# ajzhai/PEANUT

Hardware: AMD Instinct MI355X
Metric: maps/sec for 480x480x(4+N_cat) prediction fwd, batch 32 (higher is better)
Workload: dtype f32; 1 GPU; 480x480, 14-channel (4+10) partial maps -> 6-class prediction forward (PSPNet R50-V1c-D8), batch 32 per GPU, seeded random-init weights; survey_config=2, global_batch=32, parallelism=dp1 (map shards, no data-path collective)

## Files before the change

### peanut_amd/csrc/common.h

```cpp
#pragma once
#include <hip/hip_runtime.h>
#include <stdint.h>
#include <string>

namespace peanut {

void set_error(const std::string& msg);
int fail(int code, const std::string& msg);
void note_kernel(const char* family);
const char* noted_kernel();

#define PEANUT_HIP_CHECK(expr)                                                            \
  do {                                                                                    \
    hipError_t _e = (expr);                                                               \
    if (_e != hipSuccess)                                                                 \
      return ::peanut::fail(-3, std::string(#expr) + ": " + hipGetErrorString(_e));       \
  } while (0)

struct ConvDesc {
  int cin;
  int cout;
  int kh, kw, stride, pad, dil;
  int relu;
  int bn_tile;
// ... 49 lines not shown
#pragma clang fp contract(off)
  const float gx = ((float)x + 0.5f - bx[0]) / (bx[2] - bx[0]) * 2.f - 1.f;
  const float gy = ((float)y + 0.5f - bx[1]) / (bx[3] - bx[1]) * 2.f - 1.f;
  const float ix = ((gx + 1.f) * (float)M - 1.f) / 2.f, iy = ((gy + 1.f) * (float)M - 1.f) / 2.f;
  const float fx = floorf(ix), fy = floorf(iy);
  const int x0 = (int)fminf(fmaxf(fx, -2.f), (float)M + 1.f), y0 = (int)fminf(fmaxf(fy, -2.f), (float)M + 1.f);
  if (x0 < -1 || x0 >= M || y0 < -1 || y0 >= M) return 0.f;
  const float lx = ix - fx, ly = iy - fy;
  const float wx = 1.f - lx, wy = 1.f - ly;
  auto at = [&](int yy, int xx) -> float {
    return ((unsigned)yy < (unsigned)M && (unsigned)xx < (unsigned)M) ? m[yy * M + xx] : 0.f;
  };
  return at(y0, x0) * wy * wx + at(y0, x0 + 1) * wy * lx + at(y0 + 1, x0) * ly * wx + at(y0 + 1, x0 + 1) * ly * lx;
}

inline int conv_out_dim(int n, int k, int s, int p, int d) { return (n + 2 * p - d * (k - 1) - 1) / s + 1; }

void conv_pick_tiles(int cin_pad, int cout, int* bn_tile, int* bk, bool pointwise = false);
size_t conv_packed_floats(int cin_pad, int cout, int kh, int kw, int bn_tile);
void pack_conv_weights(const float* w_oihw, int cout, int cin_real, int cin_pad, int kh, int kw,
                       int bn_tile, int bk, float* out);
int launch_conv(const ConvDesc& d, const ConvArgs& a, hipStream_t stream);
bool conv_pw_enabled();
bool conv_pw_uses_256(int cout, long long M, int mt_per_group, int bn_tile, int cin);
int conv_pw_256_min_k();
bool conv_pw_uses_256w(int cout, long long M, int mt_per_group, int bn_tile, int cin, int flush_ktiles);
bool conv_pw_narrow_tiles(int cin, int cout, long long M, int bn_tile, int mt_per_group);
bool conv_pw_uses_256p(int cout, long long M, int mt_per_group, int bn_tile, int cin, int flush_ktiles, long long in_pixels = 0);
struct ConvKParams;
bool gemm_skinny_takes(const ConvKParams& p, int bn_tile, size_t ws_floats);
int launch_gemm_skinny(const ConvKParams& p, float* ws, size_t ws_floats, hipStream_t stream);
bool conv_pw_uses_256wp(int cout, long long M, int stride, int mt_per_group, int bn_tile, int c1, int c2, int flush_ktiles);
bool conv_pw_uses_ares(int cin, int cout, long long M, int stride, bool two_source, int flush_ktiles, int bn_tile);

bool conv_patch_eligible(const ConvDesc& d, const ConvArgs& a);
const char* conv_patch_kernel_name(const ConvDesc& d, bool nchw);
bool conv_patch_nchw_eligible(const ConvDesc& d, int B, int Ho, int Wo, int creal);
int launch_conv_patch_nchw(const ConvDesc& d, const float* x_nchw, int creal, float* y, int B, int H, int W, int Ho, int Wo, hipStream_t stream);

void wino_geometry(int B, int H, int W, int dil, int* th, int* tw, long long* n_tiles, long long* m_pad, int gran = 128, int m = 4);
void wino_transform_weights(const float* w_oihw, int cout, int cin, float* out, int m = 4);
int launch_wino_input(const float* x, float* V, int B, int H, int W, int C, int dil, hipStream_t s, int gran = 128, int m = 4, long long m_pad_total = 0,
                      const DeferredSplit* df = nullptr);
bool wino_input_accepts_deferred(int B, int H, int W, int C, int dil, int gran, int m);
long long wino_deferred_count();
int launch_wino_output(const float* Mb, const float* scale, const float* shift, const float* res, float* y,
                       int B, int H, int W, int C, int dil, int relu, hipStream_t s, int gran = 128, int m = 4, long long m_pad_total = 0);

bool gemm_rs_uses_256(int cout, long long M, int mt_per_group, int bn_tile, int cin);
const char* gemm_rs_kernel_name(int cout, long long M, int mt_per_group, int bn_tile, int cin, int planes);
size_t sx_packed_bytes(int cin_pad, int cout, int bn_tile, int planes);
void pack_weights_sx(const float* w, int cout, int cin_real, int cin_pad, int bn_tile, int planes, float wscale, void* out);
float sx_pack_scale(const float* w, size_t n, int planes);
size_t sx_conv_packed_bytes(int cin_pad, int cout, int kh, int kw, int bn_tile, int planes);
void pack_weights_sx_conv(const float* w_oihw, int cout, int cin_real, int cin_pad, int kh, int kw, int bn_tile, int planes,
                          float wscale, void* out);

int launch_nchw_to_nhwc_pad(const float* x, float* y, int B, int C, int H, int W, int Cpad, hipStream_t s);
int launch_maxpool3x3s2(const float* x, float* y, int B, int H, int W, int C, int Ho, int Wo, hipStream_t s);
int launch_ppm_pool(const float* x, float* out, int B, int H, int W, int C, const int* scales, int nscales,
                    hipStream_t s, int scale_rows = 0);
size_t ppm_pool_scratch_floats(int B, int H, int C, const int* scales, int nscales);
int launch_ppm_pool2(const float* x, float* scratch, float* out, int B, int H, int W, int C, const int* scales,
                     int nscales, hipStream_t s, int scale_rows = 0);
int launch_ppm_upsample_concat(const float* table, float* out, int B, int H, int W, int Cp, const int* scales,
                               int nscales, int align_corners, hipStream_t s);
// ... 7 lines not shown
```

### peanut_amd/csrc/conv_common.h

```cpp
#pragma once
#include <stdlib.h>

#include <atomic>

#include "common.h"
#include "options.h"

namespace peanut {

typedef float f32x16 __attribute__((ext_vector_type(16)));
typedef float f32x4 __attribute__((ext_vector_type(4)));

__device__ __forceinline__ float relu_keep_nan(float v) { return v < 0.f ? 0.f : v; }
__device__ __forceinline__ f32x4 relu_keep_nan(f32x4 v) {
  return f32x4{relu_keep_nan(v.x), relu_keep_nan(v.y), relu_keep_nan(v.z), relu_keep_nan(v.w)};
}

struct ConvKParams {
  const float* x;
  const float* x2;
  const float* w;
  const float* scale;
  const float* shift;
  const float* res;
// ... 14 lines not shown
  int ares_pbn;
  int phase_shift;
  int sk_units, sk_maxp, sk_g, sk_q;
  int pack_bn;
  int group_valid;
  int p_order;
  float* dump;
  int stagger;
  int flush;
  DeferredSplit* defer;
  const int* group_rows;
};

template <int I>
struct IC { static constexpr int value = I; };
template <int N, int I = 0, class F>
__device__ __forceinline__ void static_for(F&& f) {
  if constexpr (I < N) {
    f(IC<I>{});
    static_for<N, I + 1>(f);
  }
}

struct KIter {
  int tap, ky, kx, cbase;
  const float* wtile;
};


const float* zero_page();
bool conv_pw_enabled();
int launch_conv_pw(const ConvKParams& p, int bn_tile, float* ws, size_t ws_floats, hipStream_t stream);
int launch_conv_pw_ares(const ConvKParams& p, int bn_tile, hipStream_t stream);
int launch_conv_pw256p(const ConvKParams& p, float* ws, size_t ws_floats, hipStream_t stream);
int launch_conv_pw256wp(const ConvKParams& p, float* ws, size_t ws_floats, hipStream_t stream);
int launch_conv_patch(const ConvKParams& p, const ConvDesc& d, int B, hipStream_t stream);
int launch_gemm_rs(const ConvKParams& p, int bn_tile, int planes, float* ws, size_t ws_floats, hipStream_t stream);
int launch_conv_rs(const ConvKParams& p, int bn_tile, int planes, float* ws, size_t ws_floats, hipStream_t stream);


struct Work { int mt, nt, kt0, kt1, item; };

__host__ __device__ __forceinline__ int sk_owner(long long U, int G, long long u) {
  int w = (int)(u * G / U);
  while (w + 1 < G && U * (w + 1) / G <= u) ++w;
  while (w > 0 && U * w / G > u) --w;
  return w;
}

__device__ __forceinline__ void tile_to_mn(const ConvKParams& p, int tile, int* mt_out, int* nt_out) {
  int mt, nt;
  if (p.nchunk > 0 && p.ntiles > p.nchunk) {
    const int full = p.ntiles / p.nchunk, rem = p.ntiles - full * p.nchunk;
    const int per_chunk = p.mtiles * p.nchunk;
    if (tile < full * per_chunk) {
      const int c = tile / per_chunk, r = tile - c * per_chunk;
      mt = r / p.nchunk;
      nt = c * p.nchunk + (r - mt * p.nchunk);
    } else {
      const int r = tile - full * per_chunk;
      mt = r / rem;
      nt = full * p.nchunk + (r - mt * rem);
    }
  } else {
    mt = tile / p.ntiles;
    nt = tile - mt * p.ntiles;
// ... 212 lines not shown
    for (int s = 1; s < parts; ++s) v += *reinterpret_cast<const f32x4*>(base + (size_t)s * (BM * BN) + row * BN + c4);
    const int ss_off = (p.mt_per_group && p.ss_group_stride) ? (mt / p.mt_per_group) * p.ss_group_stride : 0;
    const f32x4 sc = *reinterpret_cast<const f32x4*>(p.scale + ss_off + n) * p.alpha;
    const f32x4 sh = *reinterpret_cast<const f32x4*>(p.shift + ss_off + n);
#pragma unroll
    for (int e = 0; e < 4; ++e) v[e] = __builtin_fmaf(v[e], sc[e], sh[e]);
    const size_t o = (size_t)m * p.cout + n;
    if (vec_ok) {
      if (n < p.cout) {
        if (p.res) v += *reinterpret_cast<const f32x4*>(p.res + o);
        if (p.relu) v = relu_keep_nan(v);
        *reinterpret_cast<f32x4*>(p.y + o) = v;
      }
    } else {
      for (int e = 0; e < 4; ++e) {
        if (n + e < p.cout) {
          float x = v[e];
          if (p.res) x += p.res[o + e];
          if (p.relu) x = relu_keep_nan(x);
          p.y[o + e] = x;
        }
      }
    }
  }
}

struct SlotCache {
  static constexpr int kMaxDevices = 16;
  std::atomic<int> slots[kMaxDevices];
  std::atomic<int> cus[kMaxDevices];
  SlotCache() { for (int i = 0; i < kMaxDevices; ++i) { slots[i].store(0); cus[i].store(0); } }
};

template <typename KernelT, int BM, int BN, int NT = 256>
int launch_with_tail_split(KernelT kernel, ConvKParams p, float* ws, size_t ws_floats, hipStream_t stream, SlotCache* cache) {
  int dev = 0;
  if (hipGetDevice(&dev) != hipSuccess || dev < 0 || dev >= SlotCache::kMaxDevices) return fail(-3, "conv launch: no current device");
  int slots = cache->slots[dev].load(std::memory_order_relaxed), cus = cache->cus[dev].load(std::memory_order_relaxed);
  if (slots == 0) {
    int occ = 0;
    if (hipDeviceGetAttribute(&cus, hipDeviceAttributeMultiprocessorCount, dev) != hipSuccess ||
        hipOccupancyMaxActiveBlocksPerMultiprocessor(&occ, kernel, NT, 0) != hipSuccess || occ < 1)
      slots = -1;
    else
      slots = cus * occ;
    cache->cus[dev].store(cus, std::memory_order_relaxed);
    cache->slots[dev].store(slots, std::memory_order_relaxed);
  }
  const int mtiles = (p.M + BM - 1) / BM;
  const int T = mtiles * p.ntiles;
  int sp = 1;
  const int t = plan_tail_split(T, slots, cus, p.nkt, (size_t)BM * BN, ws ? ws_floats : 0, &sp);
  p.split_p = sp;
  p.n_sp = t * sp;
  p.n_full = T - t;
  p.partial = ws;
  p.mtiles = mtiles;
  p.nchunk = (int)opt(OPT_NCHUNK);
  p.res_prefetch = opt(OPT_RES_PREFETCH) != 0;
  bool deferred = false;
  if (p.defer) {
    DeferredSplit* df = p.defer;
    if (BM == 128 && BN == 128 && t > 0 && t == T && !p.res && p.mt_per_group == 0 && p.cout % 128 == 0 &&
        !(p.nchunk > 0 && p.ntiles > p.nchunk)) {
      df->valid = true;
      df->partial = ws; df->split_p = sp; df->ntiles = p.ntiles; df->M = p.M; df->cout = p.cout; df->relu = p.relu;
      df->scale = p.scale; df->shift = p.shift; df->alpha = p.alpha;
      deferred = true;
    }
    p.defer = nullptr;
  }
  hipLaunchKernelGGL(kernel, dim3((unsigned)(p.n_full + p.n_sp)), dim3(NT), 0, stream, p);
  if (t > 0 && !deferred) hipLaunchKernelGGL((conv_splitk_reduce_kernel<BM, BN>), dim3((unsigned)t, BM / 16), dim3(256), 0, stream, p);
  hipError_t e = hipGetLastError();
  if (e != hipSuccess) return fail(-3, std::string("conv launch: ") + hipGetErrorString(e));
  return 0;
}

}
```

### peanut_amd/csrc/conv_pw.hip

```cpp
#include <stdlib.h>

#include "common.h"
#include "conv_common.h"

namespace peanut {

namespace {

typedef const __attribute__((address_space(1))) void* gptr_t;
typedef __attribute__((address_space(3))) void* lptr_t;

template <int BN, int WM, int WN>
__global__ __launch_bounds__(256) __attribute__((amdgpu_waves_per_eu(BN == 128 ? 2 : (BN == 64 ? 3 : 4))))
void conv_pw_glds_kernel(const ConvKParams p) {
  constexpr int BM = 128, BK = 32;
  constexpr int TM = BM / WM, TN = BN / WN;
  constexpr int MI = TM / 32, NI = TN / 32;
  constexpr int A_FLOATS = BM * BK, B_FLOATS = BN * BK, STAGE = A_FLOATS + B_FLOATS;
  constexpr int A_INSTR = BM / 32, B_INSTR = BN / 32;
  constexpr int CS = BN + 4;
  constexpr int EP = (BM * CS > 2 * STAGE) ? WM : 1;
  constexpr int ER = BM / EP;
  constexpr int SMEM_FLOATS = (2 * STAGE > ER * CS) ? 2 * STAGE : ER * CS;
  static_assert(WM * WN == 4 && TM % 32 == 0 && TN % 32 == 0, "4 waves, wave tile a multiple of 32x32");
// ... 357 lines not shown
    _Pragma("unroll") for (int t = 0; t < MI; ++t) af[j][t] = *reinterpret_cast<const f32x4*>(cur + a_row + t * 32 * BK + sw[(g) + j]); \
    _Pragma("unroll") for (int u = 0; u < NI; ++u) bf[j][u] = *reinterpret_cast<const f32x4*>(cur + b_row + u * 32 * BK + sw[(g) + j]); \
  }
#define PW256W_MFMA_PAIR()                                                                                \
  _Pragma("unroll") for (int j = 0; j < 2; ++j)                                                           \
    _Pragma("unroll") for (int kk = 0; kk < 4; ++kk)                                                      \
      _Pragma("unroll") for (int t = 0; t < MI; ++t)                                                      \
        _Pragma("unroll") for (int u = 0; u < NI; ++u)                                                    \
          acc[t][u] = __builtin_amdgcn_mfma_f32_32x32x2f32(af[j][t][kk], bf[j][u][kk], acc[t][u], 0, 0, 0);
  for (int kt = 0; kt < nk; ++kt) {
    const float* const cur = smem + (kt & 1) * STAGE;
    float* const fill = smem + ((kt + 1) & 1) * STAGE;
    const bool more = kt + 1 < nk;
    if (more && !late) PW256W_DMA_TILE(fill);
    f32x4 af[2][MI], bf[2][NI];
    PW256W_READ_PAIR(0);
    PW256W_MFMA_PAIR();
    __builtin_amdgcn_sched_barrier(0);
    if (more && late) PW256W_DMA_TILE(fill);
    __builtin_amdgcn_sched_barrier(0);
    PW256W_READ_PAIR(2);
    PW256W_MFMA_PAIR();
    asm volatile("s_waitcnt vmcnt(0)" ::: "memory");
    PW256W_BARRIER();
  }
#undef PW256W_DMA_TILE
#undef PW256W_BARRIER
#undef PW256W_READ_PAIR
#undef PW256W_MFMA_PAIR
  conv_epilogue<BM, BN, WM, WN, WM, NT>(p, wk, acc, smem, m0, n0);
}

template <int BN, int WM, int WN>
int launch_pw_t(const ConvKParams& p, float* ws, size_t ws_floats, hipStream_t stream) {
  static SlotCache slots;
  return launch_with_tail_split<decltype(&conv_pw_glds_kernel<BN, WM, WN>), 128, BN>(&conv_pw_glds_kernel<BN, WM, WN>, p, ws,
                                                                                      ws_floats, stream, &slots);
}

}

bool conv_pw_enabled() { return opt(OPT_PW_GLDS) != 0; }

int conv_pw_256_min_k() { return (int)opt(OPT_PW256_MINK); }
bool conv_pw_uses_256(int cout, long long M, int mt_per_group, int bn_tile, int cin) {
  const long long min_tiles = opt(OPT_PW256_MINTILES);
  return bn_tile == 128 && cin >= conv_pw_256_min_k() && mt_per_group % 2 == 0 && M * cout >= min_tiles * 256 * 128;
}

bool conv_pw_uses_256w(int cout, long long M, int mt_per_group, int bn_tile, int cin, int flush) {
  const int min_k = (int)opt(OPT_PW256W_MINK);
  const long long min_tiles = opt(OPT_PW256W_MINTILES);
  return min_k > 0 && bn_tile == 128 && cout % 256 == 0 && mt_per_group == 0 && flush == 0 && cin >= min_k &&
         ((M + 255) / 256) * (cout / 256) >= min_tiles;
}

bool conv_pw_narrow_tiles(int cin, int cout, long long M, int bn_tile, int mt_per_group) {
  (void)mt_per_group;
  if (bn_tile != 128 || cin > opt(OPT_BN64_MAXK) || cout % 128 != 0) return false;
  return ((M + 127) / 128) * (cout / 128) < opt(OPT_PW64_MAXTILES);
}

int launch_conv_pw(const ConvKParams& p, int bn_tile, float* ws, size_t ws_floats, hipStream_t stream) {
  const int phase_shift_w = opt(OPT_PW256_PHASE) != 0;
  if (gemm_skinny_takes(p, bn_tile, ws ? ws_floats : 0)) return launch_gemm_skinny(p, ws, ws_floats, stream);
  if (conv_pw_uses_256wp(p.cout, p.M, p.stride, p.mt_per_group, bn_tile, p.c1, p.c2, p.flush)) {
    const int rc = launch_conv_pw256wp(p, ws, ws_floats, stream);
    if (rc != 1) return rc;
  }
  if (conv_pw_uses_ares(p.c1, p.cout, p.M, p.stride, p.c2 != 0, p.flush, bn_tile)) return launch_conv_pw_ares(p, bn_tile, stream);
  if (conv_pw_uses_256w(p.cout, p.M, p.mt_per_group, bn_tile, p.c1 + p.c2, p.flush)) {
    static SlotCache slots256w;
    ConvKParams q = p;
    q.ntiles = p.cout / 256;
    q.phase_shift = phase_shift_w;
    note_kernel("conv_pw_glds_256x256");
    return launch_with_tail_split<decltype(&conv_pw_glds256w_kernel), 256, 256, 512>(&conv_pw_glds256w_kernel, q, ws, ws_floats, stream,
                                                                                      &slots256w);
  }
  if (conv_pw_uses_256p(p.cout, p.M, p.mt_per_group, bn_tile, p.c1 + p.c2, p.flush, (long long)(p.M / p.HoWo) * p.H * p.W) && !(p.flush && p.res)) {
    const int rc = launch_conv_pw256p(p, ws, ws_floats, stream);
    if (rc != 1) return rc;
  }
  if (conv_pw_uses_256(p.cout, p.M, p.mt_per_group, bn_tile, p.c1 + p.c2)) {
    static SlotCache slots256;
    ConvKParams q = p;
    if (q.mt_per_group) q.mt_per_group /= 2;
    q.phase_shift = phase_shift_w;
    if (opt(OPT_PW256_SKIP_PAD) == 0) q.group_valid = 0;
    note_kernel("conv_pw_glds_256x128");
    return launch_with_tail_split<decltype(&conv_pw_glds256_kernel), 256, 128, 512>(&conv_pw_glds256_kernel, q, ws, ws_floats, stream,
                                                                                     &slots256);
  }
  if (conv_pw_narrow_tiles(p.c1 + p.c2, p.cout, p.M, bn_tile, p.mt_per_group)) {
    ConvKParams q = p;
    q.pack_bn = 128;
    q.ntiles = p.ntiles * 2;
    note_kernel("conv_pw_glds_128x64");
    return launch_pw_t<64, 2, 2>(q, ws, ws_floats, stream);
  }
  note_kernel(bn_tile == 128 ? "conv_pw_glds_128x128" : (bn_tile == 64 ? "conv_pw_glds_128x64" : "conv_pw_glds_128x32"));
  if (bn_tile == 128) return launch_pw_t<128, 2, 2>(p, ws, ws_floats, stream);
  if (bn_tile == 64) return launch_pw_t<64, 2, 2>(p, ws, ws_floats, stream);
// ... 6 lines not shown
```

### peanut_amd/csrc/options.h

```cpp
#pragma once
#include <stdlib.h>
#include <string.h>

#include <string>

namespace peanut {

enum OptionId {
  OPT_PW_GLDS, OPT_PW256_MINK, OPT_PW256_MINTILES, OPT_PW256_PHASE, OPT_PW256_SKIP_PAD, OPT_PW256W_MINK, OPT_PW256W_MINTILES, OPT_PW256P_MINK, OPT_PW256P_MINTILES, OPT_PW256P_FLUSH, OPT_PW256P_ORDER, OPT_PW256P_STREAMK, OPT_PW256WP_MINK, OPT_PW256WP_MINTILES, OPT_PW256WP_NPRE, OPT_PW256WP_STAGGER, OPT_PW_ARES, OPT_PW_SKINNY,
  OPT_PW_ARES_MINUNITS, OPT_PATCH_MINTILES, OPT_STEM_NCHW, OPT_BN64_MAXK, OPT_PW_BN64_MAXK, OPT_PW64_MAXTILES, OPT_FP32_BK, OPT_NCHUNK, OPT_RES_PREFETCH, OPT_SPLIT_MODEL,
  OPT_RS_CONV, OPT_RS_BN64_MAXK, OPT_RS256_MINK, OPT_RS256_MINTILES, OPT_RS64_MAXK, OPT_RS64_MAXTILES,
  OPT_WINO_M, OPT_WINO_HEAD_M, OPT_WINO6_MAXDIL, OPT_WINO5_MINDIL, OPT_WINO_FLUSH_CH, OPT_WINO_MIN_CIN, OPT_WINO_NARROW_MINPIX, OPT_WINO_SMALL_MAXWG, OPT_DEFER_SPLITK,
  OPT_PPM_OVERLAP, OPT_PPM_GROUPED, OPT_PPM_TERM_ROWS, OPT_PPM_GROUP_ROWS, OPT_RCNN_WINO_M, OPT_RCNN_STEM_S2D, OPT_RCNN_RPN_FUSED, OPT_RCNN_FPN_OVERLAP, OPT_RCNN_RANK_SORT, OPT_RCNN_TOPK_SLICE, OPT_RCNN_NMS_LEVELS, OPT_FMM_LOCAL32, OPT_FMM_MAX_PASSES, OPT_FMM_BLOCKED, OPT_FMM_INNER,
  OPT_COUNT
};

struct OptionInfo {
  const char* key;
  long long def;
  bool upload_time;
  const char* help;
};

inline const OptionInfo* option_table() {
  static const OptionInfo t[OPT_COUNT] = {
      {"pw_glds", 1, false, "fp32 1x1 convs / grouped GEMMs on the LDS-DMA kernels of conv_pw.hip (0: conv_igemm)"},
      {"pw256_mink", 1024, false, "fewest input channels for the 256 x 128 three-stage kernel"},
      {"pw256_mintiles", 256, false, "fewest 256 x 128 tiles for that kernel"},
      {"pw256_phase", 1, false, "the two waves of a SIMD request their LDS-DMA pieces half an iteration apart"},
      {"pw256_skip_pad", 1, false, "256 x 128 kernel, grouped GEMMs: waves whose rows are all group padding issue no MFMAs (0: compute the zero rows)"},
      {"pw256w_mink", 768, false, "fewest input channels for the 256 x 256 two-stage kernel (0: off)"},
      {"pw256w_mintiles", 1536, false, "fewest 256 x 256 tiles for that kernel"},
      {"pw256p_mink", 512, false, "fewest input channels for the persistent 256 x 128 kernel (conv_pw256p.hip; 0: off)"},
      {"pw256p_mintiles", 512, false, "fewest 256 x 128 tiles for that kernel"},
      {"pw256p_flush", 512, false, "most input channels of a Winograd position GEMM (two-level accumulation) that runs on the persistent kernel (0: none)"},
      {"pw256p_order", 1, false, "persistent 256 x 128 kernel: 1 = the workgroups of an XCD walk its run of tiles side by side (neighbours share operand panels in L2), 0 = one contiguous run per workgroup"},
      {"pw256p_streamk", 1, false, "persistent 256 x 128 kernel: the tail tiles' k-tiles as one stream in equal runs per workgroup (0: every tail tile cut into the same number of parts)"},
      {"pw256wp_mink", 512, false, "fewest input channels for the persistent 256 x 256 kernel (conv_pw256wp.hip; 0: off)"},
      {"pw256wp_mintiles", 768, false, "fewest 256 x 256 tiles for that kernel"},
      {"pw256wp_npre", 0, false, "persistent 256 x 256 kernel: accumulator blocks per in-place epilogue group (2 or 4; 0 = two with a residual, four without)"},
      {"pw256wp_stagger", 0, false, "persistent 256 x 256 kernel: spread of the workgroups' start times in sleeps of ~3.4 us (their tile boundaries -- 512 KiB of epilogue traffic per CU -- then fall at different times)"},
      {"pw_ares", 1, false, "K = 128 / 256 pointwise layers on the persistent A-resident kernel (conv_pw_ares.hip)"},
      {"pw_skinny", 1, false, "grouped pointwise launches with at most 64 data rows per group (the PSP pyramid's per-scale convs and Q tables at batch 1) on the skinny weight-streaming kernel (gemm_skinny.hip: 6 KiB of LDS, fits next to any other kernel; 0: the MFMA kernels on 128-row padded tiles)"},
      {"pw_ares_minunits", 512, false, "fewest (m-tile, n-tile) units for that kernel"},
      {"patch_mintiles", 1024, false, "3x3 convs of 16 / 32 input channels on the persistent LDS-patch kernel (conv_patch.hip) from this many 8 x 16 output tiles (0: off)"},
      {"stem_nchw", 1, false, "prediction forward: the first stem conv reads the NCHW input itself (conv_patch.hip, NCHW variant) instead of a layout pass + NHWC conv (fp32 mode, when the patch kernel takes the layer)"},
      {"bn64_maxk", 256, true, "128 x 64 tiles for layers with at most this many input channels"},
      {"pw_bn64_maxk", 128, true, "pointwise layers / Winograd position GEMMs: weights PACKED 64 wide up to this many input channels (wider layers: 128-wide packing, 64-wide tiles chosen per shape)"},
      {"pw64_maxtiles", 512, false, "a 128-wide-packed pointwise layer with at most bn64_maxk input channels runs 128 x 64 tiles while its 128 x 128 tiling has fewer tiles than this (two per CU)"},
      {"fp32_bk", 0, true, "16: force 16-channel k-tiles in conv_igemm (experiment)"},
      {"nchunk", 8, false, "n-tiles per chunk of the tile order (0: n fastest over all n-tiles)"},
      {"res_prefetch", 1, false, "request the first residual rows before the last k-tile's MFMAs"},
      {"split_model", 1, false, "tail split-K plan counts CUs (1) or resident slots (0)"},
      {"rs_conv", 1, true, "emulated modes: non-pointwise convs on conv_rs.hip (0: fp32 MFMA kernel)"},
      {"rs_bn64_maxk", 128, true, "emulated modes: 128 x 64 tiles up to this many input channels"},
      {"rs256_mink", 512, false, "emulated modes: fewest input channels for the 256 x 256 kernel"},
      {"rs256_mintiles", 256, false, "emulated modes: fewest 256 x 256 tiles for it"},
      {"rs64_maxk", 512, false, "emulated modes: 64 x 64 tiles up to this many input channels"},
      {"rs64_maxtiles", 128, false, "emulated modes: ... and below this many 128-row tiles"},
      {"wino_m", 0, true, "4 / 5 / 6: force one Winograd form on every eligible layer (0: policy)"},
      {"wino_head_m", 0, true, "4 / 5 / 6: Winograd form of the PSP bottleneck (0: policy)"},
      {"wino6_maxdil", 4, true, "largest dilation that gets an F(6x6) form"},
      {"wino5_mindil", 4, true, "smallest dilation that also gets an F(5x5) form (0: none)"},
      {"wino_flush_ch", 64, true, "channels per partial sum of the position GEMMs' two-level accumulation (0: off)"},
      {"wino_min_cin", 0, true, "fewest input channels of a Winograd layer (0: the planner's policy)"},
      {"wino_narrow_minpix", 20000, false, "layers under 128 channels take their Winograd form from this many input pixels on (round 6: 100 000 -> 20 000 -- with the small-problem transforms one 720 x 720 map's layer1 conv2, 32 400 pixels, gains 5 us per layer as F(6x6); profiles/r9e)"},
      {"wino_small_maxwg", 1024, false, "Winograd transforms: launches with fewer workgroups than this of the one-thread-per-tile kernels take the small-problem variants (a workgroup per tile and 64-channel slice, a thread per line, through LDS; bit-identical; 0: never)"},
      {"defer_splitk", 1, false, "a Bottleneck conv1 whose every tile is split along k leaves its partial tiles unsummed and conv2's (small-problem) Winograd input transform sums them: one launch fewer per block at batch 1, bit-identical (0: every conv runs its own reduce); read when a (B, H, W) plan is built"},
      {"ppm_overlap", -1, false, "pyramid branch of the PSP head on a side stream: 0 / 1, -1 = by size"},
      {"ppm_grouped", -1, false, "per-scale PSP GEMMs as one grouped launch: 0 / 1, -1 = by size"},
      {"ppm_term_rows", 1, false, "folded pyramid term: one wave per output row, no barrier in the row loop (0: the workgroup-wide two-phase kernel)"},
      {"ppm_group_rows", 0, false, "pyramid pooling, row pass: rows added up per workgroup (1..5; 0 = by size: as many as still leave ~768 workgroups)"},
      {"rcnn_wino_m", 0, true, "detector front end: 4 / 5 / 6 pins one Winograd form (0: per shape)"},
      {"rcnn_stem_s2d", 1, true, "detector stem 7x7 stride 2 as a space-to-depth 4x4 conv"},
      {"rcnn_rpn_fused", 1, false, "detector: the RPN head on all five pyramid levels as one chain (five input transforms, ONE grouped Winograd GEMM, five output transforms, one objectness and one anchor-delta GEMM over all levels' rows: 12 launches instead of 25); read when a (B, H, W) plan is built"},
      {"rcnn_fpn_overlap", 0, false, "detector: the FPN output convs of p5, p4, p3 on a side stream next to the lateral / top-down chain that ends in p2's (round 5 experiment, bit-identical; measured SLOWER at batch 1, 5.70 against 5.61 ms per frame, profiles/r8: off); read when a (B, H, W) plan is built"},
      {"rcnn_rank_sort", 1, false, "detector: the RPN candidates of an image are ordered by counting the larger keys (n / 64 workgroups) instead of one workgroup's bitonic sort (round 5; same order: the keys are distinct)"},
// ... 61 lines not shown
```

### peanut_amd/csrc/pred_api.hip

```cpp
#include <math.h>
#include <string.h>

#include <map>
#include <memory>
#include <string>
#include <vector>

#include "net_common.h"

namespace peanut {

static thread_local std::string g_err;
void set_error(const std::string& msg) { g_err = msg; }
int fail(int code, const std::string& msg) {
  g_err = msg;
  return code;
}
static thread_local const char* g_kernel = "";
void note_kernel(const char* family) { g_kernel = family; }
const char* noted_kernel() { return g_kernel; }

namespace {

enum OpKind { OP_TO_NHWC, OP_CONV, OP_CONV_NCHW, OP_MAXPOOL, OP_PPM_POOL, OP_PPM_UP, OP_PPM_TERM, OP_UPSAMPLE, OP_WINO_IN, OP_WINO_GEMM, OP_WINO_OUT };
// ... 150 lines not shown
  const size_t wb = parts[0]->w.bytes, sb = (size_t)d0.cout_pad * sizeof(float), n = parts.size();
  if ((*rc = G->w.ensure(wb * n)) || (*rc = G->ss.ensure(2 * sb * n))) return nullptr;
  for (size_t i = 0; i < n; ++i) {
    if (hipMemcpy((char*)G->w.p + i * wb, parts[i]->w.p, wb, hipMemcpyDeviceToDevice) != hipSuccess ||
        hipMemcpy((char*)G->ss.p + i * sb, parts[i]->d.scale, sb, hipMemcpyDeviceToDevice) != hipSuccess ||
        hipMemcpy((char*)G->ss.p + (n + i) * sb, parts[i]->d.shift, sb, hipMemcpyDeviceToDevice) != hipSuccess) {
      *rc = fail(PEANUT_EHIP, name + ": grouping the per-scale layers failed");
      return nullptr;
    }
  }
  G->d.w_packed = (const float*)G->w.p;
  G->d.scale = (const float*)G->ss.p;
  G->d.shift = (const float*)G->ss.p + n * d0.cout_pad;
  G->d.w_s = nullptr;
  G->d.rs = 0;
  return G;
}

std::string conv_kernel_name(const ConvDesc& d, bool two_source = false, long long M = 0, int mt_per_group = 0, const Act* out = nullptr,
                             bool has_res = false) {
  if (out && !two_source && !has_res) {
    ConvArgs a{};
    a.B = out->B; a.Ho = out->H; a.Wo = out->W;
    if (conv_patch_eligible(d, a)) return conv_patch_kernel_name(d, false);
  }
  if (d.rs == 2) return std::string(d.s_planes == 3 ? "conv_rs6_128x" : (d.s_planes == 4 ? "conv_rs3h_128x" : "conv_rs3_128x")) + std::to_string(d.bn_tile);
  if (d.rs) return gemm_rs_kernel_name(d.cout, M, mt_per_group, d.bn_tile, d.cin, d.s_planes);
  if (d.bk == 32 && d.kh == 1 && d.kw == 1 && d.pad == 0 && (!two_source || d.stride == 1) && d.cin % 32 == 0 && conv_pw_enabled())
  {
    const int flush = d.flush_ch / d.bk;
    if (conv_pw_uses_256wp(d.cout, M, d.stride, mt_per_group, d.bn_tile, d.cin, 0, flush))
      return "conv_pw_glds_256x256p";
    if (conv_pw_uses_ares(d.cin, d.cout, M, d.stride, two_source, flush, d.bn_tile)) return "conv_pw_ares_128x128";
    if (conv_pw_uses_256w(d.cout, M, mt_per_group, d.bn_tile, d.cin, flush)) return "conv_pw_glds_256x256";
    if (conv_pw_uses_256p(d.cout, M, mt_per_group, d.bn_tile, d.cin, flush, M * d.stride * d.stride)) return "conv_pw_glds_256x128p";
    if (conv_pw_uses_256(d.cout, M, mt_per_group, d.bn_tile, d.cin)) return "conv_pw_glds_256x128";
    if (conv_pw_narrow_tiles(d.cin, d.cout, M, d.bn_tile, mt_per_group)) return "conv_pw_glds_128x64";
    return "conv_pw_glds_128x" + std::to_string(d.bn_tile);
  }
  return "conv_igemm_128x" + std::to_string(d.bn_tile) + "x" + std::to_string(d.bk);
}

void push_conv(Plan& pl, const ConvLayer* L, const Act& in, const Act* in2, const Act* res, const Act& out, Arena* ar = nullptr) {
  const bool wino = L->has_wino && !in2 && ar && (long long)in.B * in.H * in.W >= wino_min_pixels(L->d.cin);
  if (wino) L = wino_pick_form(L, in.B, in.H, in.W);
  if (wino) {
    int th, tw;
    long long n_tiles, m_pad;
    const bool rs_gemm = L->wino.rs != 0;
    const int gran = wino_gran_for(*L, in.B, in.H, in.W);
    wino_geometry(in.B, in.H, in.W, L->d.dil, &th, &tw, &n_tiles, &m_pad, gran, L->wino_m);
    const double np = (double)L->wino_np();
    const long long npl = L->wino_np();
    Act v = make_act(*ar, 1, 1, (int)(npl * m_pad), in.C);
    Act m = make_act(*ar, 1, 1, (int)(npl * m_pad), L->d.cout);
    const std::string fam = L->wino_m == 6 ? "wino6_" : (L->wino_m == 5 ? "wino5_" : "wino_");
    const std::string tag = "[" + fam;
    Op a; a.kind = OP_WINO_IN; a.name = L->name + tag + "in]"; a.kernel = fam + "input"; a.conv = L; a.in = in; a.out = v;
    a.wino_gran = gran;
    a.bytes = (double)in.bytes + np * (double)n_tiles * in.C * 4.0;
    pl.ops.push_back(a);
    Op g; g.kind = OP_WINO_GEMM; g.name = L->name + tag + "gemm]"; g.kernel = conv_kernel_name(L->wino, false, npl * m_pad, (int)(m_pad / 128)); g.conv = L;
    g.in = v; g.in.W = (int)(npl * m_pad); g.in.C = in.C; g.out = m; g.wino_mt_per_group = (int)(m_pad / 128); g.wino_gran = gran; g.wino_valid_rows = (int)n_tiles;
    g.flops = 2.0 * np * (double)m_pad * L->d.cout * L->cin_real;
    g.bytes = np * (double)m_pad * (in.C * 4.0 + L->d.cout * 4.0) +
              np * (rs_gemm ? (double)L->wino_group_bytes : (double)L->wino_group_floats * 4);
// ... 729 lines not shown
```

Measured before the change: 891.7 maps/s.

## Add persistent weight-resident pointwise conv kernel for small K/N layers

Adds a persistent pointwise GEMM kernel that loads the whole weight matrix (K,N in {64,128,256}, at most 128 KiB) into LDS once per workgroup. It then streams 128-row activation tiles through a multi-stage global-to-LDS ring, and overlaps each tile's epilogue (BN scale/shift, residual, ReLU) with the next tile's MFMA work. It is meant to cut the repeated weight loads and per-tile launch overhead of the tile-per-workgroup kernels on layer1-style 1x1 convs. The cost is a large LDS footprint (one workgroup per CU), a fixed grid tied to the CU count, and a possible split-accumulation path whose results may differ slightly in rounding.

After: 894.6 maps/s (median of 6 runs). About the same (+0.3%).

```diff
diff --git a/peanut_amd/csrc/common.h b/peanut_amd/csrc/common.h
--- a/peanut_amd/csrc/common.h
+++ b/peanut_amd/csrc/common.h
@@ -105,6 +105,7 @@
 int launch_gemm_skinny(const ConvKParams& p, float* ws, size_t ws_floats, hipStream_t stream);
 bool conv_pw_uses_256wp(int cout, long long M, int stride, int mt_per_group, int bn_tile, int c1, int c2, int flush_ktiles);
 bool conv_pw_uses_ares(int cin, int cout, long long M, int stride, bool two_source, int flush_ktiles, int bn_tile);
+bool conv_pw_uses_wres(int cin, int cout, long long M, int stride, int flush_ktiles, int bn_tile, int mt_per_group);
 
 bool conv_patch_eligible(const ConvDesc& d, const ConvArgs& a);
 const char* conv_patch_kernel_name(const ConvDesc& d, bool nchw);
diff --git a/peanut_amd/csrc/conv_common.h b/peanut_amd/csrc/conv_common.h
--- a/peanut_amd/csrc/conv_common.h
+++ b/peanut_amd/csrc/conv_common.h
@@ -70,6 +70,7 @@
 bool conv_pw_enabled();
 int launch_conv_pw(const ConvKParams& p, int bn_tile, float* ws, size_t ws_floats, hipStream_t stream);
 int launch_conv_pw_ares(const ConvKParams& p, int bn_tile, hipStream_t stream);
+int launch_conv_pw_wres(const ConvKParams& p, int bn_tile, int split_from, hipStream_t stream);
 int launch_conv_pw256p(const ConvKParams& p, float* ws, size_t ws_floats, hipStream_t stream);
 int launch_conv_pw256wp(const ConvKParams& p, float* ws, size_t ws_floats, hipStream_t stream);
 int launch_conv_patch(const ConvKParams& p, const ConvDesc& d, int B, hipStream_t stream);
@@ -348,21 +349,30 @@
   SlotCache() { for (int i = 0; i < kMaxDevices; ++i) { slots[i].store(0); cus[i].store(0); } }
 };
 
-template <typename KernelT, int BM, int BN, int NT = 256>
-int launch_with_tail_split(KernelT kernel, ConvKParams p, float* ws, size_t ws_floats, hipStream_t stream, SlotCache* cache) {
+template <typename KernelT>
+bool resident_slots(KernelT kernel, int nt, SlotCache* cache, int* slots_out, int* cus_out) {
   int dev = 0;
-  if (hipGetDevice(&dev) != hipSuccess || dev < 0 || dev >= SlotCache::kMaxDevices) return fail(-3, "conv launch: no current device");
+  if (hipGetDevice(&dev) != hipSuccess || dev < 0 || dev >= SlotCache::kMaxDevices) return false;
   int slots = cache->slots[dev].load(std::memory_order_relaxed), cus = cache->cus[dev].load(std::memory_order_relaxed);
   if (slots == 0) {
     int occ = 0;
     if (hipDeviceGetAttribute(&cus, hipDeviceAttributeMultiprocessorCount, dev) != hipSuccess ||
-        hipOccupancyMaxActiveBlocksPerMultiprocessor(&occ, kernel, NT, 0) != hipSuccess || occ < 1)
+        hipOccupancyMaxActiveBlocksPerMultiprocessor(&occ, kernel, nt, 0) != hipSuccess || occ < 1)
       slots = -1;
     else
       slots = cus * occ;
     cache->cus[dev].store(cus, std::memory_order_relaxed);
     cache->slots[dev].store(slots, std::memory_order_relaxed);
   }
+  *slots_out = slots;
+  *cus_out = cus;
+  return true;
+}
+
+template <typename KernelT, int BM, int BN, int NT = 256>
+int launch_with_tail_split(KernelT kernel, ConvKParams p, float* ws, size_t ws_floats, hipStream_t stream, SlotCache* cache) {
+  int slots = 0, cus = 0;
+  if (!resident_slots(kernel, NT, cache, &slots, &cus)) return fail(-3, "conv launch: no current device");
   const int mtiles = (p.M + BM - 1) / BM;
   const int T = mtiles * p.ntiles;
   int sp = 1;
diff --git a/peanut_amd/csrc/conv_pw.hip b/peanut_amd/csrc/conv_pw.hip
--- a/peanut_amd/csrc/conv_pw.hip
+++ b/peanut_amd/csrc/conv_pw.hip
@@ -413,10 +413,23 @@
 }
 
 template <int BN, int WM, int WN>
+SlotCache* pw_slots() {
+  static SlotCache slots;
+  return &slots;
+}
+
+template <int BN, int WM, int WN>
 int launch_pw_t(const ConvKParams& p, float* ws, size_t ws_floats, hipStream_t stream) {
-  static SlotCache slots;
   return launch_with_tail_split<decltype(&conv_pw_glds_kernel<BN, WM, WN>), 128, BN>(&conv_pw_glds_kernel<BN, WM, WN>, p, ws,
-                                                                                      ws_floats, stream, &slots);
+                                                                                      ws_floats, stream, pw_slots<BN, WM, WN>());
+}
+
+int pw64_split_from(const ConvKParams& p, size_t ws_floats) {
+  int slots = 0, cus = 0, sp = 1;
+  if (!resident_slots(&conv_pw_glds_kernel<64, 2, 2>, 256, pw_slots<64, 2, 2>(), &slots, &cus)) return 0x7fffffff;
+  const int T = (p.M + 127) / 128 * p.ntiles;
+  const int t = plan_tail_split(T, slots, cus, p.nkt, (size_t)128 * 64, ws_floats, &sp);
+  return (t > 0 && sp > 1) ? T - t : 0x7fffffff;
 }
 
 }
@@ -450,6 +463,8 @@
     if (rc != 1) return rc;
   }
   if (conv_pw_uses_ares(p.c1, p.cout, p.M, p.stride, p.c2 != 0, p.flush, bn_tile)) return launch_conv_pw_ares(p, bn_tile, stream);
+  if (conv_pw_uses_wres(p.c1 + p.c2, p.cout, p.M, p.stride, p.flush, bn_tile, p.mt_per_group))
+    return launch_conv_pw_wres(p, bn_tile, p.c1 + p.c2 == 256 ? pw64_split_from(p, ws ? ws_floats : 0) : 0x7fffffff, stream);
   if (conv_pw_uses_256w(p.cout, p.M, p.mt_per_group, bn_tile, p.c1 + p.c2, p.flush)) {
     static SlotCache slots256w;
     ConvKParams q = p;
diff --git a/peanut_amd/csrc/conv_pw_wres.hip b/peanut_amd/csrc/conv_pw_wres.hip
--- /dev/null
+++ b/peanut_amd/csrc/conv_pw_wres.hip
@@ -0,0 +1,351 @@
+#include <stdlib.h>
+
+#include "common.h"
+#include "conv_common.h"
+
+namespace peanut {
+
+namespace {
+
+typedef const __attribute__((address_space(1))) void* gptr_t;
+typedef __attribute__((address_space(3))) void* lptr_t;
+
+struct WresParams {
+  ConvKParams p;
+  int pbn;
+  int split_from;
+};
+
+constexpr int wres_stages(int nk, int n) {
+  const int ch = (128 * n / 512) / nk, room = 10 - nk * n / 128;
+  int s = room < 6 ? room : 6;
+  while (s > 2 && (s - 2) * (2 + ch) > 60) --s;
+  return s;
+}
+
+template <int NK, int N, bool FLUSH, bool RES>
+__global__ __launch_bounds__(512) void conv_pw_wres_kernel(const WresParams wp) {
+  const ConvKParams& p = wp.p;
+  constexpr int BK = 32, TILE = 128 * BK;
+  constexpr int WTILE = N * BK;
+  constexpr int WM = N == 256 ? 2 : 4, WN = 8 / WM;
+  constexpr int TM = 128 / WM, TN = N / WN;
+  constexpr int MI = TM / 32, NI = TN / 32, NB = MI * NI;
+  constexpr int ACC = NB * 16;
+  constexpr int CH = ACC / NK;
+  constexpr int WPIECES = NK * N / 64;
+  constexpr int S = wres_stages(NK, N), D = S - 1;
+  constexpr int VM_DMA = (S - 2) * 2, VM_FULL = (S - 2) * (2 + CH);
+  constexpr bool SPLIT = NK == 8 && !FLUSH;
+  static_assert(NK == 2 || NK == 4 || NK == 8, "K = 64, 128 or 256");
+  static_assert(N == 64 || N == 128 || N == 256, "N = 64, 128 or 256");
+  static_assert(NK * WTILE * 4 <= 128 * 1024 && ACC % NK == 0 && S >= 2 && VM_FULL <= 63, "weights fit beside the ring; whole chunks");
+  __shared__ __attribute__((aligned(1024))) float smem[NK * WTILE + S * TILE];
+  float* const ring = smem + NK * WTILE;
+
+  const int tid = threadIdx.x, lane = tid & 63;
+  const int wave = __builtin_amdgcn_readfirstlane(tid >> 6);
+  const int lr = lane >> 3, lp = lane & 7;
+  const int wm = wave / WN, wn = wave % WN;
+  const int li = lane & 31, hi = lane >> 5;
+  const bool late = p.phase_shift && wave >= 4;
+
+  const int G = gridDim.x, bid = blockIdx.x;
+  const int lw = (bid & 7) * (G >> 3) + (bid >> 3);
+  const long long T = p.mtiles;
+  const int t0 = (int)(T * lw / G), t1 = (int)(T * (lw + 1) / G);
+  if (t0 >= t1) return;
+
+  const int pbn = wp.pbn;
+  auto dma_w = [&](int group) {
+    const float* base = p.w + (size_t)group * p.w_group_stride;
+    int wlr = lr, wlp = lp;
+    asm volatile("" : "+v"(wlr), "+v"(wlp));
+#pragma unroll
+    for (int i = 0; i < WPIECES; ++i) {
+      const int q = wave + 8 * i;
+      const int kt = q / (N / 8), r = (q % (N / 8)) * 8 + wlr;
+      const int c = wlp ^ ((r >> 1) & 7);
+      const float* src = base + (size_t)(r / pbn) * (NK * pbn * BK) + kt * (pbn * BK) + (r % pbn) * BK + c * 4;
+      __builtin_amdgcn_global_load_lds((gptr_t)src, (lptr_t)(smem + q * 256), 16, 0, 0);
+    }
+  };
+  const int k1 = p.c1 / BK;
+  auto dma_a = [&](int mt, int kt, int stage) {
+#pragma unroll
+    for (int j = 0; j < 2; ++j) {
+      const int r = (wave * 2 + j) * 8 + lr;
+      const int m = mt * 128 + r;
+      const size_t mc = (size_t)(m < p.M ? m : p.M - 1);
+      const int c = lp ^ ((r >> 1) & 7);
+      const float* src = kt < k1 ? p.x + mc * p.c1 + kt * BK + c * 4 : p.x2 + mc * p.c2 + (kt - k1) * BK + c * 4;
+      __builtin_amdgcn_global_load_lds((gptr_t)src, (lptr_t)(ring + stage * TILE + (wave * 2 + j) * 256), 16, 0, 0);
+    }
+  };
+
+  const int swz = (li >> 1) & 7;
+  int sw[4];
+#pragma unroll
+  for (int ks = 0; ks < 4; ++ks) sw[ks] = ((ks * 2 + hi) ^ swz) * 4;
+  const int a_row = (wm * TM + li) * BK;
+  const int b_row = (wn * TN + li) * BK;
+
+  f32x16 acc[NB], acc2[NB], prev[NB];
+#pragma unroll
+  for (int b = 0; b < NB; ++b)
+#pragma unroll
+    for (int r = 0; r < 16; ++r) { acc[b][r] = 0.f; acc2[b][r] = 0.f; prev[b][r] = 0.f; }
+
+  const int lane_row = wm * TM + 4 * hi, lane_col = wn * TN + li;
+  const unsigned lane_off = (unsigned)(lane_row * N + lane_col);
+  constexpr bool has_res = RES;
+  const float alpha = p.alpha;
+  const bool relu = p.relu != 0;
+  bool prev_valid = false;
+  size_t prev_el = 0;
+  float scm[NI], shv[NI];
+  auto load_ss = [&](int group) {
+    const int ss_off = (p.mt_per_group && p.ss_group_stride) ? group * p.ss_group_stride : 0;
+#pragma unroll
+    for (int u = 0; u < NI; ++u) {
+      scm[u] = p.scale[ss_off + lane_col + u * 32] * alpha;
+      shv[u] = p.shift[ss_off + lane_col + u * 32];
+    }
+  };
+
+#define WRES_ROW(idx) ((((idx) >> 4) / NI) * 32 + 8 * (((idx) & 15) >> 2) + ((idx) & 3))
+#define WRES_COL(idx) ((((idx) >> 4) % NI) * 32)
+#define WRES_VALUE(idx, r) \
+  float v = prev[(idx) >> 4][(idx) & 15] * scm[((idx) >> 4) % NI] + shv[((idx) >> 4) % NI]; \
+  if (has_res) v += (r);                                                                   \
+  if (relu) v = relu_keep_nan(v);
+#define WRES_CHUNK_LOADS(kt)                                                               \
+  float resv[CH];                                                                          \
+  _Pragma("unroll") for (int i = 0; i < CH; ++i) resv[i] = 0.f;                            \
+  if (has_res && prev_valid) {                                                             \
+    const float* const rl = p.res + prev_el + lane_off;                                    \
+    _Pragma("unroll") for (int i = 0; i < CH; ++i) {                                       \
+      const int idx = (kt) * CH + i;                                                       \
+      resv[i] = rl[WRES_ROW(idx) * N + WRES_COL(idx)];                                     \
+    }                                                                                      \
+  }
+#define WRES_CHUNK_FINISH(kt)                                                              \
+  if (prev_valid) {                                                                        \
+    float* const ol = p.y + prev_el + lane_off;                                            \
+    _Pragma("unroll") for (int i = 0; i < CH; ++i) {                                       \
+      const int idx = (kt) * CH + i;                                                       \
+      WRES_VALUE(idx, resv[i])                                                             \
+      ol[WRES_ROW(idx) * N + WRES_COL(idx)] = v;                                           \
+    }                                                                                      \
+  }
+
+  int group = p.mt_per_group ? t0 / p.mt_per_group : 0;
+  dma_w(group);
+#pragma unroll
+  for (int d = 0; d < D; ++d)
+    if (t0 + d / NK < t1) dma_a(t0 + d / NK, d % NK, d);
+  load_ss(group);
+  __builtin_amdgcn_s_waitcnt(0x0F70);
+  asm volatile("" ::: "memory");
+  __builtin_amdgcn_s_barrier();
+  asm volatile("" ::: "memory");
+
+  int stage = 0;
+  int store_iters = 0;
+  for (int mt = t0; mt < t1; ++mt) {
+    const bool nxt = mt + 1 < t1;
+    const bool split = SPLIT && mt >= wp.split_from;
+
+    static_for<NK>([&](auto kc) {
+      constexpr int kt = decltype(kc)::value;
+      const float* const cur_a = ring + stage * TILE;
+      const float* const cur_b = smem + kt * WTILE;
+      WRES_CHUNK_LOADS(kt)
+      const bool req = mt + (kt + D) / NK < t1;
+      auto request = [&]() {
+        if (req) dma_a(mt + (kt + D) / NK, (kt + D) % NK, stage == 0 ? S - 1 : stage - 1);
+      };
+      if (!late) request();
+      __builtin_amdgcn_sched_barrier(0);
+      constexpr int GR = N == 256 ? 1 : 2;
+      f32x4 af[GR][MI], bf[GR][NI];
+#define WRES_READ_GROUPS(g)                                                                                             \
+  _Pragma("unroll") for (int j = 0; j < GR; ++j) {                                                                      \
+    _Pragma("unroll") for (int t = 0; t < MI; ++t) af[j][t] = *reinterpret_cast<const f32x4*>(cur_a + a_row + t * 32 * BK + sw[(g) + j]); \
+    _Pragma("unroll") for (int u = 0; u < NI; ++u) bf[j][u] = *reinterpret_cast<const f32x4*>(cur_b + b_row + u * 32 * BK + sw[(g) + j]); \
+  }
+#define WRES_MFMA_GROUPS()                                                                                \
+  _Pragma("unroll") for (int j = 0; j < GR; ++j)                                                          \
+    _Pragma("unroll") for (int kk = 0; kk < 4; ++kk)                                                      \
+      _Pragma("unroll") for (int t = 0; t < MI; ++t)                                                      \
+        _Pragma("unroll") for (int u = 0; u < NI; ++u)                                                    \
+          acc[t * NI + u] = __builtin_amdgcn_mfma_f32_32x32x2f32(af[j][t][kk], bf[j][u][kk], acc[t * NI + u], 0, 0, 0);
+#pragma unroll
+      for (int g = 0; g < 2; g += GR) {
+        WRES_READ_GROUPS(g);
+        WRES_MFMA_GROUPS();
+      }
+      __builtin_amdgcn_sched_barrier(0);
+      if (late) request();
+      __builtin_amdgcn_sched_barrier(0);
+#pragma unroll
+      for (int g = 2; g < 4; g += GR) {
+        WRES_READ_GROUPS(g);
+        WRES_MFMA_GROUPS();
+      }
+#undef WRES_READ_GROUPS
+#undef WRES_MFMA_GROUPS
+      if (FLUSH && (kt & 1)) {
+#pragma unroll
+        for (int b = 0; b < NB; ++b) {
+          acc2[b] += acc[b];
+#pragma unroll
+          for (int r = 0; r < 16; ++r) acc[b][r] = 0.f;
+        }
+      }
+      if (SPLIT && kt == NK / 2 - 1) {
+        if (split) {
+#pragma unroll
+          for (int b = 0; b < NB; ++b) {
+            acc2[b] = acc[b];
+#pragma unroll
+            for (int r = 0; r < 16; ++r) acc[b][r] = 0.f;
+          }
+        }
+      }
+      __builtin_amdgcn_sched_barrier(0);
+      if (RES || !req || S == 2) __builtin_amdgcn_s_waitcnt(0x0F70);
+      else if (store_iters >= S - 2) __builtin_amdgcn_s_waitcnt((VM_FULL & 15) | ((VM_FULL >> 4) << 14) | 0x0F70);
+      else __builtin_amdgcn_s_waitcnt((VM_DMA & 15) | ((VM_DMA >> 4) << 14) | 0x0F70);
+      asm volatile("" ::: "memory");
+      __builtin_amdgcn_sched_barrier(0);
+      WRES_CHUNK_FINISH(kt)
+      if (prev_valid && store_iters < S) ++store_iters;
+      asm volatile("s_waitcnt lgkmcnt(0)" ::: "memory");
+      __builtin_amdgcn_s_barrier();
+      asm volatile("" ::: "memory");
+      stage = stage + 1 == S ? 0 : stage + 1;
+    });
+
+#pragma unroll
+    for (int b = 0; b < NB; ++b) {
+      if (FLUSH) prev[b] = acc2[b];
+      else if (SPLIT && split) prev[b] = acc2[b] + acc[b];
+      else prev[b] = acc[b];
+#pragma unroll
+      for (int r = 0; r < 16; ++r) { acc[b][r] = 0.f; acc2[b][r] = 0.f; }
+    }
+    prev_el = (size_t)mt * 128 * N;
+    prev_valid = true;
+    if (nxt && p.mt_per_group) {
+      const int g_n = (mt + 1) / p.mt_per_group;
+      if (g_n != group) {
+        static_for<NK>([&](auto kc) {
+          constexpr int kt = decltype(kc)::value;
+          WRES_CHUNK_LOADS(kt)
+          WRES_CHUNK_FINISH(kt)
+        });
+        prev_valid = false;
+        store_iters = 0;
+        group = g_n;
+        dma_w(group);
+        load_ss(group);
+        __builtin_amdgcn_s_waitcnt(0x0F70);
+        asm volatile("" ::: "memory");
+        __builtin_amdgcn_s_barrier();
+        asm volatile("" ::: "memory");
+      }
+    }
+  }
+
+  if (prev_valid) {
+    const int left = p.M - (t1 - 1) * 128;
+    if (left >= 128) {
+      static_for<NK>([&](auto kc) {
+        constexpr int kt = decltype(kc)::value;
+        WRES_CHUNK_LOADS(kt)
+        WRES_CHUNK_FINISH(kt)
+      });
+    } else {
+      const float* const rb = p.res + prev_el;
+      float* const ob = p.y + prev_el;
+#pragma unroll
+      for (int idx = 0; idx < ACC; ++idx) {
+        const int row = lane_row + WRES_ROW(idx);
+        if (row < left) {
+          const unsigned o = (unsigned)(row * N + lane_col + WRES_COL(idx));
+          const float r = has_res ? rb[o] : 0.f;
+          WRES_VALUE(idx, r)
+          ob[o] = v;
+        }
+      }
+    }
+  }
+#undef WRES_CHUNK_LOADS
+#undef WRES_CHUNK_FINISH
+#undef WRES_VALUE
+#undef WRES_ROW
+#undef WRES_COL
+}
+
+template <int NK, int N, bool FLUSH, bool RES>
+int launch_wres_r(const WresParams& wp, hipStream_t stream) {
+  int dev = 0, cus = 0;
+  if (hipGetDevice(&dev) != hipSuccess || hipDeviceGetAttribute(&cus, hipDeviceAttributeMultiprocessorCount, dev) != hipSuccess || cus < 8)
+    return fail(-3, "conv_pw_wres: no current device");
+  const int G = cus - cus % 8;
+  hipLaunchKernelGGL((conv_pw_wres_kernel<NK, N, FLUSH, RES>), dim3((unsigned)G), dim3(512), 0, stream, wp);
+  hipError_t e = hipGetLastError();
+  if (e != hipSuccess) return fail(-3, std::string("conv_pw_wres launch: ") + hipGetErrorString(e));
+  return 0;
+}
+
+template <int NK, int N, bool FLUSH>
+int launch_wres_t(const WresParams& wp, hipStream_t stream) {
+  return wp.p.res ? launch_wres_r<NK, N, FLUSH, true>(wp, stream) : launch_wres_r<NK, N, FLUSH, false>(wp, stream);
+}
+
+template <int NK, bool FLUSH>
+int launch_wres_n(const WresParams& wp, hipStream_t stream) {
+  const int n = wp.p.cout;
+  if constexpr (NK <= 4) {
+    if (n == 256 && !FLUSH) return launch_wres_t<NK, 256, false>(wp, stream);
+    if (n == 128) return launch_wres_t<NK, 128, FLUSH>(wp, stream);
+  }
+  if (n == 64) return launch_wres_t<NK, 64, FLUSH>(wp, stream);
+  return fail(-2, "conv_pw_wres: unsupported shape");
+}
+
+}
+
+bool conv_pw_uses_wres(int cin, int cout, long long M, int stride, int flush_ktiles, int bn_tile, int mt_per_group) {
+  if (opt(OPT_PW_WRES) == 0 || stride != 1) return false;
+  if (cin != 64 && cin != 128 && cin != 256) return false;
+  if (cout != 64 && cout != 128 && cout != 256) return false;
+  if ((long long)cin * cout * 4 > 128 * 1024) return false;
+  if (cin == 256 && (cout != 64 || mt_per_group != 0)) return false;
+  if (bn_tile != 64 && bn_tile != 128) return false;
+  if (cout % bn_tile != 0) return false;
+  if (flush_ktiles != 0 && !(flush_ktiles == 2 && cin == cout && cin <= 128)) return false;
+  if (mt_per_group != 0 && M % 128 != 0) return false;
+  return (M + 127) / 128 >= opt(OPT_PW_WRES_MINTILES);
+}
+
+int launch_conv_pw_wres(const ConvKParams& p0, int bn_tile, int split_from, hipStream_t stream) {
+  WresParams wp{};
+  wp.p = p0;
+  wp.p.phase_shift = opt(OPT_PW256_PHASE) != 0;
+  wp.p.mtiles = (p0.M + 127) / 128;
+  wp.p.defer = nullptr;
+  wp.pbn = bn_tile;
+  wp.split_from = split_from;
+  const int K = p0.c1 + p0.c2;
+  const bool flush = p0.flush == 2;
+  note_kernel(p0.cout == 64 ? "conv_pw_wres_128x64" : (p0.cout == 128 ? "conv_pw_wres_128x128" : "conv_pw_wres_128x256"));
+  if (K == 64) return flush ? launch_wres_n<2, true>(wp, stream) : launch_wres_n<2, false>(wp, stream);
+  if (K == 128) return flush ? launch_wres_n<4, true>(wp, stream) : launch_wres_n<4, false>(wp, stream);
+  if (K == 256 && !flush) return launch_wres_n<8, false>(wp, stream);
+  return fail(-2, "conv_pw_wres: unsupported shape");
+}
+
+}
diff --git a/peanut_amd/csrc/options.h b/peanut_amd/csrc/options.h
--- a/peanut_amd/csrc/options.h
+++ b/peanut_amd/csrc/options.h
@@ -8,7 +8,7 @@
 
 enum OptionId {
   OPT_PW_GLDS, OPT_PW256_MINK, OPT_PW256_MINTILES, OPT_PW256_PHASE, OPT_PW256_SKIP_PAD, OPT_PW256W_MINK, OPT_PW256W_MINTILES, OPT_PW256P_MINK, OPT_PW256P_MINTILES, OPT_PW256P_FLUSH, OPT_PW256P_ORDER, OPT_PW256P_STREAMK, OPT_PW256WP_MINK, OPT_PW256WP_MINTILES, OPT_PW256WP_NPRE, OPT_PW256WP_STAGGER, OPT_PW_ARES, OPT_PW_SKINNY,
-  OPT_PW_ARES_MINUNITS, OPT_PATCH_MINTILES, OPT_STEM_NCHW, OPT_BN64_MAXK, OPT_PW_BN64_MAXK, OPT_PW64_MAXTILES, OPT_FP32_BK, OPT_NCHUNK, OPT_RES_PREFETCH, OPT_SPLIT_MODEL,
+  OPT_PW_ARES_MINUNITS, OPT_PW_WRES, OPT_PW_WRES_MINTILES, OPT_PATCH_MINTILES, OPT_STEM_NCHW, OPT_BN64_MAXK, OPT_PW_BN64_MAXK, OPT_PW64_MAXTILES, OPT_FP32_BK, OPT_NCHUNK, OPT_RES_PREFETCH, OPT_SPLIT_MODEL,
   OPT_RS_CONV, OPT_RS_BN64_MAXK, OPT_RS256_MINK, OPT_RS256_MINTILES, OPT_RS64_MAXK, OPT_RS64_MAXTILES,
   OPT_WINO_M, OPT_WINO_HEAD_M, OPT_WINO6_MAXDIL, OPT_WINO5_MINDIL, OPT_WINO_FLUSH_CH, OPT_WINO_MIN_CIN, OPT_WINO_NARROW_MINPIX, OPT_WINO_SMALL_MAXWG, OPT_DEFER_SPLITK,
   OPT_PPM_OVERLAP, OPT_PPM_GROUPED, OPT_PPM_TERM_ROWS, OPT_PPM_GROUP_ROWS, OPT_RCNN_WINO_M, OPT_RCNN_STEM_S2D, OPT_RCNN_RPN_FUSED, OPT_RCNN_FPN_OVERLAP, OPT_RCNN_RANK_SORT, OPT_RCNN_TOPK_SLICE, OPT_RCNN_NMS_LEVELS, OPT_FMM_LOCAL32, OPT_FMM_MAX_PASSES, OPT_FMM_BLOCKED, OPT_FMM_INNER,
@@ -43,6 +43,8 @@
       {"pw_ares", 1, false, "K = 128 / 256 pointwise layers on the persistent A-resident kernel (conv_pw_ares.hip)"},
       {"pw_skinny", 1, false, "grouped pointwise launches with at most 64 data rows per group (the PSP pyramid's per-scale convs and Q tables at batch 1) on the skinny weight-streaming kernel (gemm_skinny.hip: 6 KiB of LDS, fits next to any other kernel; 0: the MFMA kernels on 128-row padded tiles)"},
       {"pw_ares_minunits", 512, false, "fewest (m-tile, n-tile) units for that kernel"},
+      {"pw_wres", 1, false, "pointwise layers / position GEMMs with K and N in {64, 128, 256} whose weight matrix fits in 128 KiB of LDS (layer1) on the persistent weight-resident kernel (conv_pw_wres.hip; 0: the tile-per-workgroup kernels)"},
+      {"pw_wres_mintiles", 512, false, "fewest 128-row tiles for that kernel (two per CU)"},
       {"patch_mintiles", 1024, false, "3x3 convs of 16 / 32 input channels on the persistent LDS-patch kernel (conv_patch.hip) from this many 8 x 16 output tiles (0: off)"},
       {"stem_nchw", 1, false, "prediction forward: the first stem conv reads the NCHW input itself (conv_patch.hip, NCHW variant) instead of a layout pass + NHWC conv (fp32 mode, when the patch kernel takes the layer)"},
       {"bn64_maxk", 256, true, "128 x 64 tiles for layers with at most this many input channels"},
diff --git a/peanut_amd/csrc/pred_api.hip b/peanut_amd/csrc/pred_api.hip
--- a/peanut_amd/csrc/pred_api.hip
+++ b/peanut_amd/csrc/pred_api.hip
@@ -206,6 +206,7 @@
     if (conv_pw_uses_256wp(d.cout, M, d.stride, mt_per_group, d.bn_tile, d.cin, 0, flush))
       return "conv_pw_glds_256x256p";
     if (conv_pw_uses_ares(d.cin, d.cout, M, d.stride, two_source, flush, d.bn_tile)) return "conv_pw_ares_128x128";
+    if (conv_pw_uses_wres(d.cin, d.cout, M, d.stride, flush, d.bn_tile, mt_per_group)) return "conv_pw_wres_128x" + std::to_string(d.cout);
     if (conv_pw_uses_256w(d.cout, M, mt_per_group, d.bn_tile, d.cin, flush)) return "conv_pw_glds_256x256";
     if (conv_pw_uses_256p(d.cout, M, mt_per_group, d.bn_tile, d.cin, flush, M * d.stride * d.stride)) return "conv_pw_glds_256x128p";
     if (conv_pw_uses_256(d.cout, M, mt_per_group, d.bn_tile, d.cin)) return "conv_pw_glds_256x128";
```
